# su1phurd/UAV-WRF-LES-PPO-LSTM

Hardware: AMD Instinct MI355X
Metric: env-steps/sec (rollout + GAE + 5-epoch PPO update), 4096 envs x 128 T per GPU, LSTM h=128 x1 (higher is better)
Workload: dtype f32

## Files before the change

### uav-wrf-les-ppo-lstm_amd/csrc/wgrad.hip

```cpp
#include <stdlib.h>
#include <type_traits>
#include "common.h"

typedef float f32x4 __attribute__((ext_vector_type(4)));

constexpr int KC = 16;

template <int H>
struct WG {
    static constexpr int NW = H / 16;
    static constexpr int NT_ = H / 16 + 1;
    static constexpr int NC = H + 16;
    static constexpr int SG = 4 * H + 16;
    static constexpr int SB = H + 16;
    static constexpr int SY = H + 16;
    static constexpr int SD = 48;
    static constexpr int BUF = KC * (SG + SB + SY + SD);
    static constexpr size_t LDS = 2 * BUF * sizeof(float);
    static constexpr size_t SLAB = (size_t)4 * H * NC + 16 * H;
};

template <int H>
__global__ __launch_bounds__(H * 4) void lstm_wgrad_kernel(
    const float* __restrict__ dgates, const float* __restrict__ y, const float* __restrict__ keep,
    const float* __restrict__ h0, const float* __restrict__ x, int I, const float* __restrict__ dheads, int NH,
    int N, int T, int64_t rows_per_block, float* __restrict__ slabs) {
    using G = WG<H>;
    constexpr int NT_ = G::NT_, SG = G::SG, SB = G::SB, SY = G::SY, SD = G::SD, BUF = G::BUF;
    extern __shared__ __attribute__((aligned(16))) float smem[];
    const int tid = threadIdx.x, lane = tid & 63, w = tid >> 6;
    const int j = lane & 15, kq = lane >> 4;
    const int64_t NTr = (int64_t)N * T;
    const int64_t r_begin = (int64_t)blockIdx.x * rows_per_block;
    const int64_t r_end = (r_begin + rows_per_block < NTr) ? r_begin + rows_per_block : NTr;
    const int nchunk = (r_end > r_begin) ? (int)((r_end - r_begin + KC - 1) / KC) : 0;

    f32x4 acc[4][NT_];
    f32x4 acch = {0.f, 0.f, 0.f, 0.f};
#pragma unroll
    for (int mi = 0; mi < 4; ++mi)
#pragma unroll
        for (int ni = 0; ni < NT_; ++ni) acc[mi][ni] = f32x4{0.f, 0.f, 0.f, 0.f};

    constexpr int GV = KC * H / (H * 4);
    float4 sg[GV];
    float4 sh, sy;
    float sx, sd;
    const int g_col4 = tid % H;
    const int g_row0 = tid / H;
    const int h_row = tid / (H / 4), h_col4 = tid % (H / 4);
    const int s_row = tid >> 3, s_f = tid & 7;

    auto load_chunk = [&](int c) {
        const int64_t base = r_begin + (int64_t)c * KC;
#pragma unroll
        for (int i = 0; i < GV; ++i) {
            const int64_t r = base + g_row0 + 4 * i;
            const float m = (r < r_end) ? 1.f : 0.f;
            const float4 v = *reinterpret_cast<const float4*>(dgates + (r < NTr ? r : NTr - 1) * (4 * H) + 4 * g_col4);
            sg[i] = make_float4(v.x * m, v.y * m, v.z * m, v.w * m);
        }
        {
            const int64_t r = base + h_row, rc = (r < NTr ? r : NTr - 1);
            const int64_t n = rc / T;
            const int t = (int)(rc - n * T);
            const float m = (r < r_end) ? 1.f : 0.f;
            const float kp = (keep ? keep[rc] : 1.f) * m;
            const float* src = (t == 0) ? (h0 + n * H) : (y + (rc - 1) * H);
            const float4 v = *reinterpret_cast<const float4*>(src + 4 * h_col4);
            sh = make_float4(v.x * kp, v.y * kp, v.z * kp, v.w * kp);
            sy = make_float4(0.f, 0.f, 0.f, 0.f);
            if (dheads) {
                const float4 u4 = *reinterpret_cast<const float4*>(y + rc * H + 4 * h_col4);
                sy = make_float4(u4.x * m, u4.y * m, u4.z * m, u4.w * m);
            }
        }
        sx = 0.f;
        sd = 0.f;
        if (tid < KC * 8) {
            const int64_t r = base + s_row;
            if (r < r_end) {
                sx = (s_f < I) ? x[r * I + s_f] : (s_f == 6 ? 1.f : 0.f);
                if (dheads && s_f < NH) sd = dheads[r * NH + s_f];
            }
        }
    };
    auto store_chunk = [&](int buf) {
        float* lg = smem + buf * BUF;
        float* lb = lg + KC * SG;
        float* ly = lb + KC * SB;
        float* ld = ly + KC * SY;
#pragma unroll
        for (int i = 0; i < GV; ++i)
            *reinterpret_cast<float4*>(lg + (g_row0 + 4 * i) * SG + 4 * g_col4) = sg[i];
        *reinterpret_cast<float4*>(lb + h_row * SB + 4 * h_col4) = sh;
        *reinterpret_cast<float4*>(ly + h_row * SY + 4 * h_col4) = sy;
        if (tid < KC * 8) {
            lb[s_row * SB + H + s_f] = sx;
            lb[s_row * SB + H + 8 + s_f] = 0.f;
            ld[s_row * SD + s_f] = sd;
            ld[s_row * SD + 8 + s_f] = 0.f;
        }
    };

    if (nchunk > 0) load_chunk(0);
    for (int c = 0; c < nchunk; ++c) {
        const int buf = c & 1;
        store_chunk(buf);
        lds_barrier();
        if (c + 1 < nchunk) load_chunk(c + 1);
        const float* lg = smem + buf * BUF;
        const float* lb = lg + KC * SG;
        const float* ly = lb + KC * SB;
        const float* ld = ly + KC * SY;
#pragma unroll
        for (int s = 0; s < KC / 4; ++s) {
            const int kr = 4 * s + kq;
            float a[4], b[NT_];
#pragma unroll
            for (int mi = 0; mi < 4; ++mi) a[mi] = lg[kr * SG + 64 * w + 16 * mi + j];
#pragma unroll
            for (int ni = 0; ni < NT_; ++ni) b[ni] = lb[kr * SB + 16 * ni + j];
            const float ah = ld[kr * SD + j];
            const float bh = ly[kr * SY + 16 * w + j];
#pragma unroll
            for (int mi = 0; mi < 4; ++mi)
#pragma unroll
                for (int ni = 0; ni < NT_; ++ni)
                    acc[mi][ni] = __builtin_amdgcn_mfma_f32_16x16x4f32(a[mi], b[ni], acc[mi][ni], 0, 0, 0);
            acch = __builtin_amdgcn_mfma_f32_16x16x4f32(ah, bh, acch, 0, 0, 0);
        }
    }
    float* slab = slabs + (size_t)blockIdx.x * G::SLAB;
#pragma unroll
    for (int mi = 0; mi < 4; ++mi)
#pragma unroll
        for (int ni = 0; ni < NT_; ++ni)
#pragma unroll
            for (int r = 0; r < 4; ++r)
                slab[(size_t)(64 * w + 16 * mi + 4 * kq + r) * G::NC + 16 * ni + j] = acc[mi][ni][r];
#pragma unroll
    for (int r = 0; r < 4; ++r) slab[(size_t)4 * H * G::NC + (size_t)(4 * kq + r) * H + 16 * w + j] = acch[r];
}


constexpr int KS6 = 32;

__device__ __forceinline__ void mac6(f32x4& d, const bf16x8 (&a)[3], const bf16x8 (&b)[3]) {
    d = __builtin_amdgcn_mfma_f32_16x16x32_bf16(a[2], b[0], d, 0, 0, 0);
    d = __builtin_amdgcn_mfma_f32_16x16x32_bf16(a[1], b[1], d, 0, 0, 0);
    d = __builtin_amdgcn_mfma_f32_16x16x32_bf16(a[0], b[2], d, 0, 0, 0);
    d = __builtin_amdgcn_mfma_f32_16x16x32_bf16(a[1], b[0], d, 0, 0, 0);
    d = __builtin_amdgcn_mfma_f32_16x16x32_bf16(a[0], b[1], d, 0, 0, 0);
    d = __builtin_amdgcn_mfma_f32_16x16x32_bf16(a[0], b[0], d, 0, 0, 0);
}

template <class P>
__device__ __forceinline__ void split8(const float (&v)[8], typename P::vec (&p)[P::NP]) {
#pragma unroll
    for (int i = 0; i < 8; ++i) {
        typename P::piece q[P::NP];
        P::split(v[i], q);
#pragma unroll
        for (int k = 0; k < P::NP; ++k) p[k][i] = q[k];
    }
}

struct WgBf16x6 {
    typedef __bf16 piece;
    typedef bf16x8 vec;
    static constexpr int NP = 3;
    static constexpr float BSCALE = 1.0f, XSCALE = 1.0f;
    static constexpr bool LOADS_BETWEEN_TILES = false;
    __device__ __forceinline__ static void split(float a, piece (&p)[NP]) { split3(a, p[0], p[1], p[2]); }
    __device__ __forceinline__ static unsigned short bits(piece v) { return bf_bits(v); }
    __device__ __forceinline__ static void mac(f32x4& d, const vec (&a)[NP], const vec (&b)[NP]) { mac6(d, a, b); }
    template <int NT_>
    __device__ __forceinline__ void split_a(int, const float (&raw)[8], vec (&ap)[NP], f32x4 (&)[NT_], int) {
        split8<WgBf16x6>(raw, ap);
    }
    __device__ __forceinline__ float row_unscale(int, int, int) const { return 1.0f; }
};

struct WgF16x3 {
    typedef _Float16 piece;
    typedef f16x8 vec;
    static constexpr int NP = 2;
    static constexpr float BSCALE = 1024.0f;
    static constexpr float XSCALE = 16.0f;
    static constexpr bool LOADS_BETWEEN_TILES = true;
    __device__ __forceinline__ static void split(float a, piece (&p)[NP]) {
        p[0] = (_Float16)a;
        p[1] = (_Float16)(a - (float)p[0]);
    }
    __device__ __forceinline__ static unsigned short bits(piece v) { return h_bits(v); }
    __device__ __forceinline__ static void mac(f32x4& d, const vec (&a)[NP], const vec (&b)[NP]) {
        d = __builtin_amdgcn_mfma_f32_16x16x32_f16(a[1], b[0], d, 0, 0, 0);
        d = __builtin_amdgcn_mfma_f32_16x16x32_f16(a[0], b[1], d, 0, 0, 0);
        d = __builtin_amdgcn_mfma_f32_16x16x32_f16(a[0], b[0], d, 0, 0, 0);
    }
    unsigned exr4 = 0xe4e4e4e4u;
    __device__ __forceinline__ int exr_get(int mi) const { return (int)((exr4 >> (8 * mi)) & 255u) - 128; }
    __device__ __forceinline__ void exr_set(int mi, int v) {
        exr4 = (exr4 & ~(255u << (8 * mi))) | ((unsigned)(v + 128) << (8 * mi));
    }
    __device__ __forceinline__ static float row_max4(float m) {
        const unsigned u = __builtin_bit_cast(unsigned, m);
        const auto s16 = __builtin_amdgcn_permlane16_swap(u, u, false, false);
        m = fmaxf(__builtin_bit_cast(float, (unsigned)s16[0]), __builtin_bit_cast(float, (unsigned)s16[1]));
        const unsigned v2 = __builtin_bit_cast(unsigned, m);
        const auto s32 = __builtin_amdgcn_permlane32_swap(v2, v2, false, false);
        return fmaxf(__builtin_bit_cast(float, (unsigned)s32[0]), __builtin_bit_cast(float, (unsigned)s32[1]));
    }
    template <int NT_>
    __device__ __forceinline__ void split_a(int mi, const float (&raw)[8], vec (&ap)[NP], f32x4 (&acc)[NT_], int kq) {
        float mx = 0.f;
#pragma unroll
        for (int e = 0; e < 8; ++e) mx = fmaxf(mx, fabsf(raw[e]));
        mx = row_max4(mx);
        const int eo = exr_get(mi);
        const int ne = mx > 0.f ? min(min(14 - __builtin_amdgcn_frexp_expf(mx), 100), eo) : eo;
        const int delta = eo - ne;
        if (__builtin_amdgcn_ballot_w64(delta != 0)) {
#pragma unroll
            for (int r = 0; r < 4; ++r) {
                const int dr = __builtin_amdgcn_ds_bpermute((4 * kq + r) * 4, delta);
                const float f = __builtin_amdgcn_ldexpf(1.0f, -dr);
#pragma unroll
                for (int ni = 0; ni < NT_; ++ni) acc[ni][r] *= f;
            }
            exr_set(mi, ne);
        }
        float sc[8];
#pragma unroll
        for (int e = 0; e < 8; ++e) sc[e] = __builtin_amdgcn_ldexpf(raw[e], ne);
        split8<WgF16x3>(sc, ap);
    }
    __device__ __forceinline__ float row_unscale(int mi, int r, int kq) const {
        const int er = __builtin_amdgcn_ds_bpermute((4 * kq + r) * 4, exr_get(mi));
        return __builtin_amdgcn_ldexpf(1.0f / BSCALE, -er);
    }
};

template <int H, class P>
struct WGS {
    static constexpr int NW = H / 16, NT = H * 4;
    static constexpr int NT_ = H / 16 + 1, NC = H + 16;
    static constexpr int KP = KS6 + 8;
    static constexpr int BPL = NC * KP, YPL = H * KP, DPL = 16 * KP;
    static constexpr int BUF = P::NP * BPL + 3 * (YPL + DPL);
    static constexpr size_t LDS = 2 * BUF * sizeof(unsigned short);
    static constexpr int XV = 16 * KS6 / NT;
    static constexpr int DV = (8 * KS6 + NT - 1) / NT;
};

#ifdef UAV_X6_PROFILE
__device__ unsigned long long g_wx6_prof[2][8];
#define WX_PROF_DECL unsigned long long pm_[8] = {0, 0, 0, 0, 0, 0, 0, 0}, pl_ = __builtin_readcyclecounter()
#define WX_PROF_MARK(i) do { const unsigned long long n_ = __builtin_readcyclecounter(); pm_[i] += n_ - pl_; pl_ = n_; } while (0)
#define WX_PROF_DEP(v) asm volatile("" ::"v"(v))
#define WX_PROF_FLUSH() do { if (blockIdx.x == 0 && lane == 0 && (w == 0 || w == H / 16 - 1)) \
        for (int i_ = 0; i_ < 8; ++i_) g_wx6_prof[w ? 1 : 0][i_] = pm_[i_]; } while (0)
extern "C" int uav_wx6_prof_read(unsigned long long* out) {
    return hipMemcpyFromSymbol(out, HIP_SYMBOL(g_wx6_prof), sizeof(g_wx6_prof)) == hipSuccess ? 0 : 1;
}
#else
#define WX_PROF_DECL
#define WX_PROF_MARK(i)
#define WX_PROF_DEP(v)
#define WX_PROF_FLUSH()
#endif

template <int H, bool HEADS, class P>
__device__ __forceinline__ void lstm_wgrad_split(
    const float* __restrict__ dgates, const float* __restrict__ y, const float* __restrict__ keep,
    const float* __restrict__ h0, const float* __restrict__ x, int I, const float* __restrict__ dheads, int NH,
    int N, int T, int rows_per_block, float* __restrict__ slabs) {
    using G = WGS<H, P>;
    using vec = typename P::vec;
    constexpr int NT_ = G::NT_, KP = G::KP, BPL = G::BPL, YPL = G::YPL, DPL = G::DPL, BUF = G::BUF, NT = G::NT;
    constexpr int XV = G::XV, DV = G::DV, NW = G::NW, NP = P::NP;
    extern __shared__ __attribute__((aligned(16))) unsigned short sm16[];
    const int tid = threadIdx.x, lane = tid & 63;
    const int w = __builtin_amdgcn_readfirstlane(tid >> 6);
    const bool late = w >= NW / 2;
    const int j = lane & 15, kq = lane >> 4;
    const int r_begin = blockIdx.x * rows_per_block;
    const int nslab = rows_per_block / KS6;
    P pol;

    const int c = tid % H;
    const int rg = __builtin_amdgcn_readfirstlane(tid / H);

    f32x4 acc[4][NT_];
    f32x4 acch = {0.f, 0.f, 0.f, 0.f};
#pragma unroll
    for (int mi = 0; mi < 4; ++mi)
#pragma unroll
        for (int ni = 0; ni < NT_; ++ni) acc[mi][ni] = f32x4{0.f, 0.f, 0.f, 0.f};

    for (int idx = tid; idx < 2 * 3 * DPL; idx += NT) {
        const int b = idx / (3 * DPL), rem = idx % (3 * DPL);
        sm16[b * BUF + NP * BPL + 3 * YPL + rem] = 0;
    }

    float raw[4][8];
    auto load_a_one = [&](int slab, int pair, int e) {
        slab = slab < nslab ? slab : nslab - 1;
        const unsigned off = (unsigned)(r_begin + slab * KS6 + 8 * kq) * (4 * H) + 64 * w + 32 * pair + 2 * j;
        const float2 t2 = *reinterpret_cast<const float2*>(dgates + (off + (unsigned)e * (4 * H)));
        raw[2 * pair][e] = t2.x;
        raw[2 * pair + 1][e] = t2.y;
    };
    auto load_a = [&](int slab, int pair) {
#pragma unroll
        for (int e = 0; e < 8; ++e) load_a_one(slab, pair, e);
    };
    constexpr int NV = HEADS ? 9 : 8;
    float v[NV], hz = 0.f, xv[XV], dv[DV];
    float kv = 1.f;
    int i_start = -1;
    auto load_b_y = [&](int slab, int i) {
        slab = slab < nslab ? slab : nslab - 1;
        const int rr = r_begin + slab * KS6 + 8 * rg - 1 + i;
        v[i] = y[(unsigned)(rr < 0 ? 0 : rr) * H + c];
    };
    auto load_b_rest = [&](int slab) {
        slab = slab < nslab ? slab : nslab - 1;
        const int q0 = r_begin + slab * KS6 + 8 * rg;
        const int tq = q0 % T;
        i_start = (tq == 0) ? 0 : (tq + 7 >= T ? T - tq : -1);
        if (i_start >= 0) hz = h0[(unsigned)((q0 + i_start) / T) * H + c];
        kv = keep ? keep[q0 + (lane & 7)] : 1.f;
#pragma unroll
        for (int k = 0; k < XV; ++k) {
            const int idx = tid + k * NT, q = idx >> 4, f = idx & 15;
            const unsigned r = (unsigned)(r_begin + slab * KS6 + q);
            xv[k] = (f < I) ? x[r * I + f] : (f == 6 ? 1.f : 0.f);
        }
#pragma unroll
        for (int k = 0; k < DV; ++k) {
            const int idx = tid + k * NT, q = idx >> 3, a = idx & 7;
            const unsigned r = (unsigned)(r_begin + slab * KS6 + (q < KS6 ? q : 0));
            dv[k] = (HEADS && a < NH && q < KS6) ? dheads[r * NH + a] : 0.f;
        }
    };
    auto load_b = [&](int slab) {
#pragma unroll
        for (int i = 0; i < NV; ++i) load_b_y(slab, i);
        load_b_rest(slab);
    };
    auto commit_b = [&](int buf) {
        unsigned short* bp = sm16 + buf * BUF;
        unsigned short* yp = bp + NP * BPL;
        unsigned short* dp = yp + 3 * YPL;
        float hp[8], yy[8];
#pragma unroll
        for (int i = 0; i < 8; ++i) {
            const float kpi = __builtin_bit_cast(float, __builtin_amdgcn_readlane(__builtin_bit_cast(int, kv), i));
            hp[i] = ((i == i_start) ? hz : v[i]) * (kpi * P::BSCALE);
            yy[i] = HEADS ? v[i + 1 < NV ? i + 1 : 0] : 0.f;
        }
        vec hq[NP];
        split8<P>(hp, hq);
#pragma unroll
        for (int p = 0; p < NP; ++p) *reinterpret_cast<vec*>(bp + p * BPL + c * KP + 8 * rg) = hq[p];
        if (HEADS) {
            bf16x8 yq[3];
            split8<WgBf16x6>(yy, yq);
#pragma unroll
            for (int p = 0; p < 3; ++p) *reinterpret_cast<bf16x8*>(yp + p * YPL + c * KP + 8 * rg) = yq[p];
        }
#pragma unroll
        for (int k = 0; k < XV; ++k) {
            const int idx = tid + k * NT, q = idx >> 4, f = idx & 15;
            typename P::piece xq[NP];
            P::split(xv[k] * P::XSCALE, xq);
            unsigned short* d = bp + (H + f) * KP + q;
#pragma unroll
            for (int p = 0; p < NP; ++p) d[p * BPL] = P::bits(xq[p]);
        }
        if (HEADS) {
#pragma unroll
            for (int k = 0; k < DV; ++k) {
                const int idx = tid + k * NT, q = idx >> 3, a = idx & 7;
                if (q < KS6) {
                    __bf16 pa, pb, pc;
                    split3(dv[k], pa, pb, pc);
                    unsigned short* d = dp + a * KP + q;
                    d[0] = bf_bits(pa);
                    d[DPL] = bf_bits(pb);
                    d[2 * DPL] = bf_bits(pc);
                }
            }
        }
    };
    vec ap[2][NP];
    auto split_pair = [&](int sl, int pair) {
#pragma unroll
        for (int m = 0; m < 2; ++m) pol.split_a(2 * pair + m, raw[2 * pair + m], ap[m], acc[2 * pair + m], kq);
        if constexpr (!P::LOADS_BETWEEN_TILES) load_a(sl + 1, pair);
    };
    auto mfma_pair = [&](int buf, int pair, int sl) {
        const unsigned short* bp = sm16 + buf * BUF;
#pragma unroll
        for (int ni = 0; ni < NT_; ++ni) {
            vec bb[NP];
            const unsigned short* src = bp + (16 * ni + j) * KP + 8 * kq;
#pragma unroll
            for (int p = 0; p < NP; ++p) bb[p] = *reinterpret_cast<const vec*>(src + p * BPL);
            P::mac(acc[2 * pair][ni], ap[0], bb);
            P::mac(acc[2 * pair + 1][ni], ap[1], bb);
            if constexpr (P::LOADS_BETWEEN_TILES) {
#pragma unroll
                for (int e = ni; e < 8; e += NT_) load_a_one(sl + 1, pair, e);
                if (pair == 1) {
#pragma unroll
                    for (int i = ni; i < NV; i += NT_) load_b_y(sl + 2, i);
                    if (ni == NT_ - 1) load_b_rest(sl + 2);
                }
                asm volatile("" ::: "memory");
            } else if (HEADS && (ni & 1)) {
                asm volatile("" ::: "memory");
            }
        }
        if (HEADS && pair == 1) {
            const unsigned short* yp = bp + NP * BPL;
            const unsigned short* dp = yp + 3 * YPL;
            bf16x8 da[3], yb[3];
            const unsigned short* sa = dp + j * KP + 8 * kq;
            const unsigned short* sb = yp + (16 * w + j) * KP + 8 * kq;
#pragma unroll
            for (int pc = 0; pc < 3; ++pc) {
                da[pc] = *reinterpret_cast<const bf16x8*>(sa + pc * DPL);
                yb[pc] = *reinterpret_cast<const bf16x8*>(sb + pc * YPL);
            }
            mac6(acch, da, yb);
        }
    };

    load_b(0);
    load_a(0, 0);
    load_a(0, 1);
    commit_b(0);
    load_b(1);
    split_pair(0, 0);
    lds_barrier();
    WX_PROF_DECL;
    for (int sl = 0; sl < nslab; ++sl) {
        const int buf = sl & 1;
        WX_PROF_MARK(0);
        mfma_pair(buf, 0, sl);
        WX_PROF_DEP(acc[0][NT_ - 1]); WX_PROF_DEP(acc[1][NT_ - 1]); WX_PROF_MARK(2);
        commit_b(buf ^ 1);
        if constexpr (!P::LOADS_BETWEEN_TILES) load_b(sl + 2);
        WX_PROF_MARK(5);
        split_pair(sl, 1);
        WX_PROF_DEP(ap[0][0]); WX_PROF_DEP(ap[1][NP - 1]); WX_PROF_MARK(3);
        mfma_pair(buf, 1, sl);
        WX_PROF_DEP(acc[2][NT_ - 1]); WX_PROF_DEP(acc[3][NT_ - 1]); WX_PROF_MARK(4);
        if (!late) { lds_barrier(); WX_PROF_MARK(7); }
        split_pair(sl + 1, 0);
        WX_PROF_DEP(ap[0][0]); WX_PROF_DEP(ap[1][NP - 1]); WX_PROF_MARK(1);
        if (late) { lds_barrier(); WX_PROF_MARK(7); }
    }
    WX_PROF_FLUSH();
    float* slab = slabs + (size_t)blockIdx.x * WG<H>::SLAB;
#pragma unroll
    for (int mi = 0; mi < 4; ++mi)
#pragma unroll
        for (int r = 0; r < 4; ++r) {
            const float usc = pol.row_unscale(mi, r, kq);
#pragma unroll
            for (int ni = 0; ni < NT_; ++ni)
                slab[(size_t)(64 * w + 32 * (mi >> 1) + 2 * (4 * kq + r) + (mi & 1)) * G::NC + 16 * ni + j] =
                    acc[mi][ni][r] * (ni == NT_ - 1 ? usc * (P::BSCALE / P::XSCALE) : usc);
        }
#pragma unroll
    for (int r = 0; r < 4; ++r) slab[(size_t)4 * H * G::NC + (size_t)(4 * kq + r) * H + 16 * w + j] = acch[r];
}

template <int H, bool HEADS>
__global__ __launch_bounds__(H * 4) void lstm_wgrad_x6_kernel(
    const float* __restrict__ dgates, const float* __restrict__ y, const float* __restrict__ keep,
    const float* __restrict__ h0, const float* __restrict__ x, int I, const float* __restrict__ dheads, int NH,
    int N, int T, int rows_per_block, float* __restrict__ slabs) {
    lstm_wgrad_split<H, HEADS, WgBf16x6>(dgates, y, keep, h0, x, I, dheads, NH, N, T, rows_per_block, slabs);
}
template <int H, bool HEADS>
__global__ __launch_bounds__(H * 4) void lstm_wgrad_h3_kernel(
    const float* __restrict__ dgates, const float* __restrict__ y, const float* __restrict__ keep,
    const float* __restrict__ h0, const float* __restrict__ x, int I, const float* __restrict__ dheads, int NH,
    int N, int T, int rows_per_block, float* __restrict__ slabs) {
    lstm_wgrad_split<H, HEADS, WgF16x3>(dgates, y, keep, h0, x, I, dheads, NH, N, T, rows_per_block, slabs);
}

template <int H>
__global__ __launch_bounds__(256) void wgrad_reduce_kernel(const float* __restrict__ slabs, int nb, int I, int NH,
                                                           float* __restrict__ dw_ih, float* __restrict__ dw_hh,
                                                           float* __restrict__ db, float* __restrict__ db_hh,
                                                           float* __restrict__ dw_head) {
    using G = WG<H>;
    const size_t o = (size_t)blockIdx.x * 256 + threadIdx.x;
    if (o >= G::SLAB) return;
    float p8[8] = {0.f, 0.f, 0.f, 0.f, 0.f, 0.f, 0.f, 0.f};
    int b = 0;
    for (; b + 8 <= nb; b += 8)
#pragma unroll
        for (int k = 0; k < 8; ++k) p8[k] += slabs[(size_t)(b + k) * G::SLAB + o];
    for (; b < nb; ++b) p8[0] += slabs[(size_t)b * G::SLAB + o];
    const float s = ((p8[0] + p8[1]) + (p8[2] + p8[3])) + ((p8[4] + p8[5]) + (p8[6] + p8[7]));
    const size_t gsz = (size_t)4 * H * G::NC;
    if (o < gsz) {
        const int m = (int)(o / G::NC), c = (int)(o % G::NC);
        if (c < H) dw_hh[(size_t)m * H + c] = s;
        else if (c - H < I) dw_ih[(size_t)m * I + (c - H)] = s;
        else if (c - H == 6) {
            db[m] = s;
            if (db_hh) db_hh[m] = s;
        }
    } else if (dw_head) {
        const int a = (int)((o - gsz) / H), uu = (int)((o - gsz) % H);
        if (a < NH) dw_head[(size_t)a * H + uu] = s;
    }
}

template <class P, int H, bool HEADS>
static constexpr auto wgrad_split_kernel() {
    if constexpr (std::is_same<P, WgF16x3>::value) return &lstm_wgrad_h3_kernel<H, HEADS>;
    else return &lstm_wgrad_x6_kernel<H, HEADS>;
}

template <class P, int H>
static int launch_wgrad_split(const float* dgates, const float* y, const float* keep, const float* h0, const float* x, int I,
                              const float* dheads, int NH, int N, int T, int nb, int rpb, float* slabs, hipStream_t st) {
    const auto kern = dheads ? wgrad_split_kernel<P, H, true>() : wgrad_split_kernel<P, H, false>();
    const size_t lds = WGS<H, P>::LDS;
    UAV_CHECK_HIP(uav_dyn_lds(reinterpret_cast<const void*>(kern), (int)lds));
    hipLaunchKernelGGL(kern, dim3(nb), dim3(H * 4), lds, st, dgates, y, keep, h0, x, I, dheads, NH, N, T, rpb, slabs);
    return 0;
}

template <int H>
static int launch_wgrad(uav_ctx* ctx, const float* dgates, const float* y, const float* keep, const float* h0,
                        const float* x, int I, const float* dheads, int NH, int N, int T,
                        float* dw_ih, float* dw_hh, float* db, float* db_hh, float* dw_head, hipStream_t st) {
    using G = WG<H>;
    const int64_t NTr = (int64_t)N * T;
    int nb = ctx->num_cu;
    const int64_t max_nb = (int64_t)(ctx->ws_bytes / (G::SLAB * sizeof(float)));
    if (nb > max_nb) nb = (int)max_nb;
    UAV_REQUIRE(nb >= 1, "uav_lstm_wgrad: workspace too small for one slab");
    int64_t rpb = (NTr + nb - 1) / nb;
    rpb = (rpb + KC - 1) / KC * KC;
    nb = (int)((NTr + rpb - 1) / rpb);
    float* slabs = (float*)ctx->ws;
    {
        int64_t rpx = (NTr + nb - 1) / nb;
        rpx = (rpx + KS6 - 1) / KS6 * KS6;
        const int nbx = (int)((NTr + rpx - 1) / rpx);
        const bool split_ok = (NTr % rpx == 0) && T >= 8 && I <= 6 && (!dheads || NH <= 8) && NTr * 4 * H < (1ll << 30) &&
                              !uav_want_f32_mfma();
        if (split_ok) {
            const int rc = uav_want_bf16x6()
                               ? launch_wgrad_split<WgBf16x6, H>(dgates, y, keep, h0, x, I, dheads, NH, N, T, nbx, (int)rpx, slabs, st)
                               : launch_wgrad_split<WgF16x3, H>(dgates, y, keep, h0, x, I, dheads, NH, N, T, nbx, (int)rpx, slabs, st);
            if (rc) return rc;
            hipLaunchKernelGGL((wgrad_reduce_kernel<H>), dim3((unsigned)((G::SLAB + 255) / 256)), dim3(256), 0, st, slabs,
                               nbx, I, NH, dw_ih, dw_hh, db, db_hh, dw_head);
            UAV_LAUNCH_CHECK();
            return 0;
        }
    }
    UAV_CHECK_HIP(uav_dyn_lds(reinterpret_cast<const void*>(&lstm_wgrad_kernel<H>), (int)G::LDS));
    hipLaunchKernelGGL((lstm_wgrad_kernel<H>), dim3(nb), dim3(H * 4), G::LDS, st, dgates, y, keep, h0, x, I, dheads, NH, N,
                       T, rpb, slabs);
    hipLaunchKernelGGL((wgrad_reduce_kernel<H>), dim3((unsigned)((G::SLAB + 255) / 256)), dim3(256), 0, st, slabs, nb, I,
                       NH, dw_ih, dw_hh, db, db_hh, dw_head);
    UAV_LAUNCH_CHECK();
    return 0;
}

int lstm_wgrad_fused(uav_ctx* ctx, const float* dgates, const float* y, const float* keep, const float* h0,
                     const float* x, int I, const float* dheads, int NH, int N, int T, int H,
                     float* dw_ih, float* dw_hh, float* db, float* db_hh, float* dw_head, hipStream_t st) {
    switch (H) {
        case 64: return launch_wgrad<64>(ctx, dgates, y, keep, h0, x, I, dheads, NH, N, T, dw_ih, dw_hh, db, db_hh, dw_head, st);
        case 128: return launch_wgrad<128>(ctx, dgates, y, keep, h0, x, I, dheads, NH, N, T, dw_ih, dw_hh, db, db_hh, dw_head, st);
    }
    uav_set_error("lstm_wgrad_fused: H=%d unsupported", H);
    return 2;
}
```

Measured before the change: 74.89 million.

## Store wgrad B operand row-major in LDS and read via ds_read_tr16 transpose

```diff
diff --git a/uav-wrf-les-ppo-lstm_amd/csrc/wgrad.hip b/uav-wrf-les-ppo-lstm_amd/csrc/wgrad.hip
--- a/uav-wrf-les-ppo-lstm_amd/csrc/wgrad.hip
+++ b/uav-wrf-les-ppo-lstm_amd/csrc/wgrad.hip
@@ -246,13 +246,34 @@
 struct WGS {
     static constexpr int NW = H / 16, NT = H * 4;
     static constexpr int NT_ = H / 16 + 1, NC = H + 16;
+    static constexpr int SR = NC;
     static constexpr int KP = KS6 + 8;
-    static constexpr int BPL = NC * KP, YPL = H * KP, DPL = 16 * KP;
+    static constexpr int BPL = KS6 * SR + 3 * 64, YPL = BPL, DPL = 16 * KP;
     static constexpr int BUF = P::NP * BPL + 3 * (YPL + DPL);
     static constexpr size_t LDS = 2 * BUF * sizeof(unsigned short);
+    static constexpr int C4 = H / 4;
+    static constexpr int RPW = 64 / C4;
     static constexpr int XV = 16 * KS6 / NT;
     static constexpr int DV = (8 * KS6 + NT - 1) / NT;
 };
+
+template <int SR>
+__device__ __forceinline__ int wg_roff(int r) { return r * SR + 64 * (r >> 3); }
+
+template <class P>
+__device__ __forceinline__ void split4(const f32x4& v, uint2 (&o)[P::NP]) {
+    typedef typename P::piece pv4 __attribute__((ext_vector_type(4)));
+    pv4 b[P::NP];
+#pragma unroll
+    for (int i = 0; i < 4; ++i) {
+        typename P::piece q[P::NP];
+        P::split(v[i], q);
+#pragma unroll
+        for (int k = 0; k < P::NP; ++k) b[k][i] = q[k];
+    }
+#pragma unroll
+    for (int k = 0; k < P::NP; ++k) o[k] = __builtin_bit_cast(uint2, b[k]);
+}
 
 #ifdef UAV_X6_PROFILE
 __device__ unsigned long long g_wx6_prof[2][8];
@@ -278,9 +299,14 @@
     int N, int T, int rows_per_block, float* __restrict__ slabs) {
     using G = WGS<H, P>;
     using vec = typename P::vec;
-    constexpr int NT_ = G::NT_, KP = G::KP, BPL = G::BPL, YPL = G::YPL, DPL = G::DPL, BUF = G::BUF, NT = G::NT;
-    constexpr int XV = G::XV, DV = G::DV, NW = G::NW, NP = P::NP;
+    constexpr int NT_ = G::NT_, KP = G::KP, SR = G::SR, BPL = G::BPL, YPL = G::YPL, DPL = G::DPL, BUF = G::BUF, NT = G::NT;
+    constexpr int XV = G::XV, DV = G::DV, NW = G::NW, NP = P::NP, C4 = G::C4, RPW = G::RPW;
+    typedef __attribute__((address_space(3))) unsigned short lds_u16;
+    typedef short v4s __attribute__((__vector_size__(4 * sizeof(short))));
+    typedef short v8s __attribute__((__vector_size__(8 * sizeof(short))));
+    typedef __attribute__((address_space(3))) v4s lds_v4s;
     extern __shared__ __attribute__((aligned(16))) unsigned short sm16[];
+    lds_u16* const s3 = (lds_u16*)sm16;
     const int tid = threadIdx.x, lane = tid & 63;
     const int w = __builtin_amdgcn_readfirstlane(tid >> 6);
     const bool late = w >= NW / 2;
@@ -289,8 +315,8 @@
     const int nslab = rows_per_block / KS6;
     P pol;
 
-    const int c = tid % H;
-    const int rg = __builtin_amdgcn_readfirstlane(tid / H);
+    const int c4 = tid % C4;
+    const int q = tid / C4;
 
     f32x4 acc[4][NT_];
     f32x4 acch = {0.f, 0.f, 0.f, 0.f};
@@ -307,8 +333,8 @@
     float raw[4][8];
     auto load_a_one = [&](int slab, int pair, int e) {
         slab = slab < nslab ? slab : nslab - 1;
-        const unsigned off = (unsigned)(r_begin + slab * KS6 + 8 * kq) * (4 * H) + 64 * w + 32 * pair + 2 * j;
-        const float2 t2 = *reinterpret_cast<const float2*>(dgates + (off + (unsigned)e * (4 * H)));
+        const unsigned off = (unsigned)(r_begin + slab * KS6 + 8 * kq + e) * (4 * H) + 64 * w + 32 * pair + 2 * j;
+        const float2 t2 = *reinterpret_cast<const float2*>(dgates + off);
         raw[2 * pair][e] = t2.x;
         raw[2 * pair + 1][e] = t2.y;
     };
@@ -316,78 +342,86 @@
 #pragma unroll
         for (int e = 0; e < 8; ++e) load_a_one(slab, pair, e);
     };
-    constexpr int NV = HEADS ? 9 : 8;
-    float v[NV], hz = 0.f, xv[XV], dv[DV];
-    float kv = 1.f;
-    int i_start = -1;
-    auto load_b_y = [&](int slab, int i) {
+    f32x4 bh[2], by[2];
+    float kv = 1.f, xv[XV], dv[DV];
+    int bn = (r_begin + q) / T, bt = r_begin + q - bn * T;
+    auto load_b_row = [&](int slab, int u) {
         slab = slab < nslab ? slab : nslab - 1;
-        const int rr = r_begin + slab * KS6 + 8 * rg - 1 + i;
-        v[i] = y[(unsigned)(rr < 0 ? 0 : rr) * H + c];
+        const int r = r_begin + slab * KS6 + q + 16 * u;
+        int n = bn, t = bt + 16 * u;
+        while (t >= T) { t -= T; ++n; }
+        const float* hs = (t == 0) ? h0 + (unsigned)n * H : y + (unsigned)(r - 1) * H;
+        bh[u] = *reinterpret_cast<const f32x4*>(hs + 4 * c4);
+        if (HEADS) by[u] = *reinterpret_cast<const f32x4*>(y + (unsigned)r * H + 4 * c4);
     };
     auto load_b_rest = [&](int slab) {
+        if (slab < nslab - 1) {
+            bt += KS6;
+            while (bt >= T) { bt -= T; ++bn; }
+        }
         slab = slab < nslab ? slab : nslab - 1;
-        const int q0 = r_begin + slab * KS6 + 8 * rg;
-        const int tq = q0 % T;
-        i_start = (tq == 0) ? 0 : (tq + 7 >= T ? T - tq : -1);
-        if (i_start >= 0) hz = h0[(unsigned)((q0 + i_start) / T) * H + c];
-        kv = keep ? keep[q0 + (lane & 7)] : 1.f;
+        const int q0 = r_begin + slab * KS6;
+        if (keep) kv = keep[q0 + (lane & 31)];
 #pragma unroll
         for (int k = 0; k < XV; ++k) {
-            const int idx = tid + k * NT, q = idx >> 4, f = idx & 15;
-            const unsigned r = (unsigned)(r_begin + slab * KS6 + q);
+            const int idx = tid + k * NT, qq = idx >> 4, f = idx & 15;
+            const unsigned r = (unsigned)(q0 + qq);
             xv[k] = (f < I) ? x[r * I + f] : (f == 6 ? 1.f : 0.f);
         }
 #pragma unroll
         for (int k = 0; k < DV; ++k) {
-            const int idx = tid + k * NT, q = idx >> 3, a = idx & 7;
-            const unsigned r = (unsigned)(r_begin + slab * KS6 + (q < KS6 ? q : 0));
-            dv[k] = (HEADS && a < NH && q < KS6) ? dheads[r * NH + a] : 0.f;
+            const int idx = tid + k * NT, qq = idx >> 3, a = idx & 7;
+            const unsigned r = (unsigned)(q0 + (qq < KS6 ? qq : 0));
+            dv[k] = (HEADS && a < NH && qq < KS6) ? dheads[r * NH + a] : 0.f;
         }
     };
     auto load_b = [&](int slab) {
-#pragma unroll
-        for (int i = 0; i < NV; ++i) load_b_y(slab, i);
+        load_b_row(slab, 0);
+        load_b_row(slab, 1);
         load_b_rest(slab);
     };
     auto commit_b = [&](int buf) {
         unsigned short* bp = sm16 + buf * BUF;
         unsigned short* yp = bp + NP * BPL;
         unsigned short* dp = yp + 3 * YPL;
-        float hp[8], yy[8];
-#pragma unroll
-        for (int i = 0; i < 8; ++i) {
-            const float kpi = __builtin_bit_cast(float, __builtin_amdgcn_readlane(__builtin_bit_cast(int, kv), i));
-            hp[i] = ((i == i_start) ? hz : v[i]) * (kpi * P::BSCALE);
-            yy[i] = HEADS ? v[i + 1 < NV ? i + 1 : 0] : 0.f;
-        }
-        vec hq[NP];
-        split8<P>(hp, hq);
-#pragma unroll
-        for (int p = 0; p < NP; ++p) *reinterpret_cast<vec*>(bp + p * BPL + c * KP + 8 * rg) = hq[p];
-        if (HEADS) {
-            bf16x8 yq[3];
-            split8<WgBf16x6>(yy, yq);
-#pragma unroll
-            for (int p = 0; p < 3; ++p) *reinterpret_cast<bf16x8*>(yp + p * YPL + c * KP + 8 * rg) = yq[p];
+#pragma unroll
+        for (int u = 0; u < 2; ++u) {
+            const int row = q + 16 * u;
+            float kp = 1.f;
+#pragma unroll
+            for (int s = 0; s < RPW; ++s) {
+                const float ks = __builtin_bit_cast(float, __builtin_amdgcn_readlane(__builtin_bit_cast(int, kv), RPW * w + s + 16 * u));
+                kp = (lane / C4 == s) ? ks : kp;
+            }
+            kp *= P::BSCALE;
+            uint2 hq[NP];
+            split4<P>(f32x4{bh[u][0] * kp, bh[u][1] * kp, bh[u][2] * kp, bh[u][3] * kp}, hq);
+#pragma unroll
+            for (int p = 0; p < NP; ++p) *reinterpret_cast<uint2*>(bp + p * BPL + wg_roff<SR>(row) + 4 * c4) = hq[p];
+            if (HEADS) {
+                uint2 yq[3];
+                split4<WgBf16x6>(by[u], yq);
+#pragma unroll
+                for (int p = 0; p < 3; ++p) *reinterpret_cast<uint2*>(yp + p * YPL + wg_roff<SR>(row) + 4 * c4) = yq[p];
+            }
         }
 #pragma unroll
         for (int k = 0; k < XV; ++k) {
-            const int idx = tid + k * NT, q = idx >> 4, f = idx & 15;
+            const int idx = tid + k * NT, qq = idx >> 4, f = idx & 15;
             typename P::piece xq[NP];
             P::split(xv[k] * P::XSCALE, xq);
-            unsigned short* d = bp + (H + f) * KP + q;
+            unsigned short* d = bp + wg_roff<SR>(qq) + H + f;
 #pragma unroll
             for (int p = 0; p < NP; ++p) d[p * BPL] = P::bits(xq[p]);
         }
         if (HEADS) {
 #pragma unroll
             for (int k = 0; k < DV; ++k) {
-                const int idx = tid + k * NT, q = idx >> 3, a = idx & 7;
-                if (q < KS6) {
+                const int idx = tid + k * NT, qq = idx >> 3, a = idx & 7;
+                if (qq < KS6) {
                     __bf16 pa, pb, pc;
                     split3(dv[k], pa, pb, pc);
-                    unsigned short* d = dp + a * KP + q;
+                    unsigned short* d = dp + a * KP + qq;
                     d[0] = bf_bits(pa);
                     d[DPL] = bf_bits(pb);
                     d[2 * DPL] = bf_bits(pc);
@@ -395,6 +429,13 @@
             }
         }
     };
+    const int tr_off = wg_roff<SR>(8 * kq + ((lane >> 2) & 3)) + 4 * (lane & 3);
+    auto tr_frag = [&](const lds_u16* base) {
+        const v4s lo = __builtin_amdgcn_ds_read_tr16_b64_v4i16((lds_v4s*)(base + tr_off));
+        const v4s hi = __builtin_amdgcn_ds_read_tr16_b64_v4i16((lds_v4s*)(base + tr_off + 4 * SR));
+        const v8s r = {lo[0], lo[1], lo[2], lo[3], hi[0], hi[1], hi[2], hi[3]};
+        return r;
+    };
     vec ap[2][NP];
     auto split_pair = [&](int sl, int pair) {
 #pragma unroll
@@ -402,21 +443,19 @@
         if constexpr (!P::LOADS_BETWEEN_TILES) load_a(sl + 1, pair);
     };
     auto mfma_pair = [&](int buf, int pair, int sl) {
-        const unsigned short* bp = sm16 + buf * BUF;
+        const lds_u16* bp = s3 + buf * BUF;
 #pragma unroll
         for (int ni = 0; ni < NT_; ++ni) {
             vec bb[NP];
-            const unsigned short* src = bp + (16 * ni + j) * KP + 8 * kq;
-#pragma unroll
-            for (int p = 0; p < NP; ++p) bb[p] = *reinterpret_cast<const vec*>(src + p * BPL);
+#pragma unroll
+            for (int p = 0; p < NP; ++p) bb[p] = __builtin_bit_cast(vec, tr_frag(bp + p * BPL + 16 * ni));
             P::mac(acc[2 * pair][ni], ap[0], bb);
             P::mac(acc[2 * pair + 1][ni], ap[1], bb);
             if constexpr (P::LOADS_BETWEEN_TILES) {
 #pragma unroll
                 for (int e = ni; e < 8; e += NT_) load_a_one(sl + 1, pair, e);
                 if (pair == 1) {
-#pragma unroll
-                    for (int i = ni; i < NV; i += NT_) load_b_y(sl + 2, i);
+                    if (ni < 2) load_b_row(sl + 2, ni);
                     if (ni == NT_ - 1) load_b_rest(sl + 2);
                 }
                 asm volatile("" ::: "memory");
@@ -425,15 +464,14 @@
             }
         }
         if (HEADS && pair == 1) {
-            const unsigned short* yp = bp + NP * BPL;
-            const unsigned short* dp = yp + 3 * YPL;
+            const lds_u16* yp = bp + NP * BPL;
+            const unsigned short* dp = sm16 + buf * BUF + NP * BPL + 3 * YPL;
             bf16x8 da[3], yb[3];
             const unsigned short* sa = dp + j * KP + 8 * kq;
-            const unsigned short* sb = yp + (16 * w + j) * KP + 8 * kq;
 #pragma unroll
             for (int pc = 0; pc < 3; ++pc) {
                 da[pc] = *reinterpret_cast<const bf16x8*>(sa + pc * DPL);
-                yb[pc] = *reinterpret_cast<const bf16x8*>(sb + pc * YPL);
+                yb[pc] = __builtin_bit_cast(bf16x8, tr_frag(yp + pc * YPL + 16 * w));
             }
             mac6(acch, da, yb);
         }
@@ -465,19 +503,21 @@
         if (late) { lds_barrier(); WX_PROF_MARK(7); }
     }
     WX_PROF_FLUSH();
+    const int lane_e = (int)__builtin_amdgcn_mbcnt_hi(~0u, __builtin_amdgcn_mbcnt_lo(~0u, 0u));
+    const int je = lane_e & 15, kqe = lane_e >> 4;
     float* slab = slabs + (size_t)blockIdx.x * WG<H>::SLAB;
 #pragma unroll
     for (int mi = 0; mi < 4; ++mi)
 #pragma unroll
         for (int r = 0; r < 4; ++r) {
-            const float usc = pol.row_unscale(mi, r, kq);
+            const float usc = pol.row_unscale(mi, r, kqe);
 #pragma unroll
             for (int ni = 0; ni < NT_; ++ni)
-                slab[(size_t)(64 * w + 32 * (mi >> 1) + 2 * (4 * kq + r) + (mi & 1)) * G::NC + 16 * ni + j] =
+                slab[(size_t)(64 * w + 32 * (mi >> 1) + 2 * (4 * kqe + r) + (mi & 1)) * G::NC + 16 * ni + je] =
                     acc[mi][ni][r] * (ni == NT_ - 1 ? usc * (P::BSCALE / P::XSCALE) : usc);
         }
 #pragma unroll
-    for (int r = 0; r < 4; ++r) slab[(size_t)4 * H * G::NC + (size_t)(4 * kq + r) * H + 16 * w + j] = acch[r];
+    for (int r = 0; r < 4; ++r) slab[(size_t)4 * H * G::NC + (size_t)(4 * kqe + r) * H + 16 * w + je] = acch[r];
 }
 
 template <int H, bool HEADS>
```

Result: no change. 75.76 million (median of 6 runs) (+1.2%).
